# bipul-mohanto/OptixPathTracer

Measured on AMD Instinct MI355X. Metric: Mrays/s (and ms/frame) at 1080p 4spp depth8; 1/2/4/8 MI355X scaling, higher is better.
Workload: dtype f32

## Files before the change

### optixpathtracer_amd/csrc/pt_bvh8.h

```cpp
#pragma once
#ifdef PT_BVH8_NODE_ONLY
#include "pt_bvh.h"
#else
#include "pt_kernels.h"
#endif

struct Node8 {
    float4 n0, n1, n2, n3, n4;
};
#ifndef PT8_LEAF_MAX
#define PT8_LEAF_MAX 3
#endif
static_assert(PT8_LEAF_MAX >= 1 && PT8_LEAF_MAX <= 3, "leafbits holds 3 bits per slot");

PT_DEV float u8f(uint32_t v, int k) { return (float)((v >> (8 * k)) & 0xffu); }

struct Bvh8Dev {
    const Node8* nodes;
    const LeafTri* tris;
    float hit_pad;
};

struct NodeHdr {
    float ox, oy, oz, sx, sy, sz;
    uint32_t imask, child_base, tri_base;
    uint32_t lbits;
};
PT_DEV NodeHdr node_hdr(const float4 n0, const float4 n1) {
    NodeHdr n;
    const uint32_t e01 = __float_as_uint(n0.w), e2m = __float_as_uint(n1.w);
    n.ox = n0.x; n.oy = n0.y; n.oz = n0.z;
    n.sx = __uint_as_float(e01 << 16); n.sy = __uint_as_float(e01 & 0xffff0000u); n.sz = __uint_as_float(e2m << 16);
    n.imask = e2m >> 16;
    n.child_base = __float_as_uint(n1.x);
    n.tri_base = __float_as_uint(n1.y);
    n.lbits = __float_as_uint(n1.z);
    return n;
}
PT_DEV uint32_t leaf_pending(uint32_t hm, uint32_t lbits) {
    uint32_t sp3 = (hm | (hm << 8)) & 0x00F00Fu;
    sp3 = (sp3 | (sp3 << 4)) & 0x0C30C3u;
    sp3 = (sp3 | (sp3 << 2)) & 0x249249u;
    return (sp3 * 7u) & lbits;
}
PT_DEV uint32_t leaf_of(uint32_t tri_base, uint32_t lbits, uint32_t bit) { return tri_base + (uint32_t)__popc(lbits & ((1u << bit) - 1u)); }
PT_DEV uint32_t leaf_first(uint32_t tri_base, uint32_t lbits, uint32_t s) { return leaf_of(tri_base, lbits, 3u * s); }
PT_DEV uint32_t leaf_count(uint32_t lbits, uint32_t s) { return (uint32_t)__popc((lbits >> (3u * s)) & 7u); }

#ifndef PT_BVH8_NODE_ONLY
#ifndef PT8_LDS_DEPTH
#define PT8_LDS_DEPTH 10
#endif
#define PT8_OVF_DEPTH 52
#ifndef PT8_REFILL
#define PT8_REFILL 40
#endif
#ifndef PT8_TRI_BIAS
#define PT8_TRI_BIAS 2
#endif
#ifndef PT8_MIN_CHUNK
#define PT8_MIN_CHUNK 64
#endif
#define PT8_CHUNK 512
#ifndef PT8_WAVES_PER_EU
#define PT8_WAVES_PER_EU 5
#endif
#ifndef PT8_STEAL_PERIOD
#define PT8_STEAL_PERIOD 3
#endif

#define PT8_WAVE_SYNC() do { __builtin_amdgcn_fence(__ATOMIC_SEQ_CST, "wavefront"); __builtin_amdgcn_wave_barrier(); } while (0)

#define PT_WAVELOG_CAP (1u << 20)
#ifdef PT_DEBUG_STATS
#define PT_STAT(x) x
#else
#define PT_STAT(x)
#endif
#if defined(PT_DEBUG_STATS) || defined(PT_DEBUG_WAVELOG)
#define PT_WLOG(x) x
#else
#define PT_WLOG(x)
#endif

#define PT_WSTRIDE 16
struct Trace8Args {
    PathState st;
    Bvh8Dev bvh;
    QView queue;
    QView queue2;
    uint32_t* work;
    uint32_t* ovf;
    int cull_back;
    unsigned long long* dbg;
    int bounce;
    int lds_skip;
    int ovf_depth;
    uint32_t* fault;
    uint32_t num_nodes;
};

#if __HIP_DEVICE_COMPILE__
typedef __attribute__((address_space(3))) uint32_t* Lds32;
typedef __attribute__((address_space(1))) uint32_t* Global32;
#else
typedef uint32_t* Lds32;
typedef uint32_t* Global32;
#endif

template <int MODE, bool LOCAL, bool CARRY = false>
PT_DEV void trace8_wave(const Trace8Args& a, const uint32_t wid, const uint32_t nw, const uint32_t ln1, const uint32_t ln2, const uint32_t woff) {
    __shared__ uint32_t s_stack[PT8_LDS_DEPTH * 2 * 64];
    __shared__ uint32_t s_prefix[PT_NSUB + 1];
    __shared__ uint32_t s_prefix2[PT_NSUB + 1];
    __shared__ unsigned long long s_key[64];
    __shared__ uint32_t s_cnt[64];
    __shared__ int32_t s_leaf[64];
    __shared__ uint32_t s_vlane[64];
    const uint32_t lane = threadIdx.x;
    const uint32_t gtid = blockIdx.x * 64u + lane;
    const uint32_t gstride = gridDim.x * 64u;
    const int lds_depth = PT8_LDS_DEPTH - a.lds_skip;
    const uint32_t n1 = LOCAL ? ln1 : qreader_init(a.queue, s_prefix);
    const uint32_t n2 = (MODE == TR_UNIFIED) ? (LOCAL ? ln2 : qreader_init(a.queue2, s_prefix2)) : 0u;
    const uint32_t n = n1 + n2;
    uint32_t chunk = (n / (nw * 2u)) & ~(uint32_t)(PT8_MIN_CHUNK < 64 ? PT8_MIN_CHUNK - 1 : 63);
    chunk = chunk < (uint32_t)PT8_MIN_CHUNK ? (uint32_t)PT8_MIN_CHUNK : (chunk > (uint32_t)PT8_CHUNK ? (uint32_t)PT8_CHUNK : chunk);
    if (LOCAL) chunk = n;
    const bool no_share = (unsigned long long)wid * chunk >= n;
    const uint32_t nchunks = (n + chunk - 1u) / chunk;
    if (no_share) return;
    uint32_t chunk_next = wid * chunk;
    uint32_t chunk_end = (chunk_next + chunk < n) ? chunk_next + chunk : n;
    const unsigned long long lt_mask = (1ull << lane) - 1ull;
    bool shadow_lane = (MODE == TR_SHADOW_APPLY);

    bool active = false, exhausted = false;
    RaySetup r;
    r.o = r.d = r.idir = r.dn = mk3(0.f);
    float tmin = 0.f, tmax = 0.f, best = 0.f;
    int32_t bprim = -1;
    int32_t bleaf = -1;
    uint32_t pm = 0;
    uint32_t g_base = 0, g_imask = 0, g_hits = 0;
    uint32_t t_base = 0, t_mask = 0, t_bits = 0;
    int sp = 0;
    bool stealing = false;
    uint32_t misc = lane;
#define OWNER (misc & 0xffu)
#define SB ((int)(misc >> 24))
#define SET_OWNER(v) (misc = (misc & ~0xffu) | (uint32_t)(v))
#define SET_SB(v) (misc = (misc & 0x00ffffffu) | ((uint32_t)(v) << 24))
    uint32_t slot = 0;
    bool unwritten = false;
    PT_STAT(uint32_t c_nodes = 0; uint32_t c_tris = 0; uint32_t c_maxsp = 0; uint32_t c_push = 0; uint32_t c_ray = 0; uint32_t c_raymax = 0; uint32_t c_iters = 0;
            uint32_t c_act = 0; uint32_t c_exec = 0; uint32_t c_nodeit = 0;)
    PT_WLOG(const unsigned long long w_t0 = wall_clock64(); unsigned long long w_tex = 0; uint32_t w_iters = 0;)
    PT_WLOG(unsigned long long w_cw = 0; unsigned long long w_cr = 0; unsigned long long w_cs = 0; uint32_t w_np = 0;)
    PT_WLOG(unsigned long long w_c01 = 0; unsigned long long w_c12 = 0; unsigned long long w_c23 = 0; const unsigned long long w_c0 = clock64();)

    const char* const node_bytes = reinterpret_cast<const char*>(a.bvh.nodes);
    const char* const tri_bytes = reinterpret_cast<const char*>(a.bvh.tris);
    const Lds32 lds_stack = (Lds32)s_stack;
    const Global32 ovf_stack = (Global32)a.ovf;
    auto push = [&](uint32_t v0, uint32_t v1) {
        PT_STAT(++c_push; if ((uint32_t)sp + 1 > c_maxsp) c_maxsp = sp + 1;)
        if (sp < lds_depth) {
            lds_stack[(sp * 2) * 64 + lane] = v0;
            lds_stack[(sp * 2 + 1) * 64 + lane] = v1;
            ++sp;
        } else if (sp < lds_depth + a.ovf_depth) {
            ovf_stack[(size_t)((sp - lds_depth) * 2) * gstride + gtid] = v0;
            ovf_stack[(size_t)((sp - lds_depth) * 2 + 1) * gstride + gtid] = v1;
            ++sp;
        } else {
            atomicOr(a.fault, 1u);
        }
    };
    auto pop = [&](uint32_t& v0, uint32_t& v1) {
        --sp;
        if (sp < lds_depth) {
            v0 = lds_stack[(sp * 2) * 64 + lane];
            v1 = lds_stack[(sp * 2 + 1) * 64 + lane];
        } else {
            v0 = ovf_stack[(size_t)((sp - lds_depth) * 2) * gstride + gtid];
            v1 = ovf_stack[(size_t)((sp - lds_depth) * 2 + 1) * gstride + gtid];
            __builtin_amdgcn_s_waitcnt(0x0f70);
        }
    };
    auto write_result = [&](float rbest, int32_t rprim) {
        if (MODE == TR_SHADOW_APPLY || (MODE == TR_UNIFIED && shadow_lane)) {
            const bool occluded = rprim != 0;
            if (MODE == TR_UNIFIED && CARRY) {
                st_st<PT_NT_TRACE_ST>(&a.st.svis[slot], occluded ? 0u : 1u);
                return;
            }
            const uint32_t ps = (MODE == TR_UNIFIED ? a.queue2 : a.queue).base[slot];
            if (a.st.vis) {
                if (!occluded) atomicOr(&a.st.vis[ps], 1u << a.bounce);
                return;
            }
            const float4 pe = st_ld<PT_NT_TRACE_LD>(&a.st.shPend[slot]);
            const int kind = __float_as_int(pe.w);
            if (kind == PEND_ALPHA) {
                if (occluded) {
                    const float4 x = a.st.alpha[ps];
                    a.st.alpha[ps] = make_float4(x.x + pe.x, x.y + pe.y, x.z + pe.z, 0.f);
                }
            } else if (!occluded) {
                float4* acc = (kind == PEND_DIRECT) ? a.st.direct : a.st.indirect;
                const float4 x = st_ld<PT_NT_TRACE_LD>(&acc[ps]);
                st_st<PT_NT_TRACE_ST>(&acc[ps], make_float4(x.x + pe.x, x.y + pe.y, x.z + pe.z, 0.f));
            }
        } else {
            st_st<PT_NT_TRACE_ST>(&a.st.hit[slot], make_float2(rbest, __int_as_float(rprim)));
        }
    };
    const auto is_shadow = [&]() { return MODE == TR_SHADOW_APPLY || MODE == TR_ANY_QUERY || (MODE == TR_UNIFIED && shadow_lane); };
    auto local_key = [&]() -> unsigned long long {
        if (is_shadow()) return bprim != 0 ? 0ull : ~0ull;
        return ((unsigned long long)__float_as_uint(best) << 32) | (unsigned long long)(uint32_t)bprim;
    };
    auto finish = [&]() {
        if (stealing) {
            atomicMin(&s_key[OWNER], local_key());
            if (atomicSub(&s_cnt[OWNER], 1u) == 1u) {
                const unsigned long long k = s_key[OWNER];
                if (is_shadow()) write_result(0.f, k == 0ull ? 1 : 0);
                else write_result(__uint_as_float((uint32_t)(k >> 32)), (int32_t)(uint32_t)k < 0 ? -1 : s_leaf[OWNER]);
            }
            active = false;
            return;
        }
        unwritten = true;
        active = false;
        PT_STAT(if (c_ray > c_raymax) c_raymax = c_ray;
                if (a.dbg) atomicAdd(&a.dbg[(is_shadow() ? 32 : 16) + (31 - __clz((int)(c_ray | 1u)))], 1ull);
                c_ray = 0;)
    };

    auto start_ray = [&](float ox, float oy, float oz, float dx, float dy, float dz) {
        r.o = mk3(ox, oy, oz);
        r.d = mk3(dx, dy, dz);
        r.idir = mk3(__builtin_amdgcn_rcpf(dx), __builtin_amdgcn_rcpf(dy), __builtin_amdgcn_rcpf(dz));
        r.dn = scl3(r.d, 1.0f / dot3(r.d, r.d));
        if (!(fabsf(dx) > 1e-30f)) r.idir.x = copysignf(1e30f, dx);
        if (!(fabsf(dy) > 1e-30f)) r.idir.y = copysignf(1e30f, dy);
        if (!(fabsf(dz) > 1e-30f)) r.idir.z = copysignf(1e30f, dz);
        pm = ((__float_as_uint(dz) >> 31) ? 0xF0u : 0x0Fu) | (((__float_as_uint(dy) >> 31) ? 0xCCu : 0x33u) << 8) | (((__float_as_uint(dx) >> 31) ? 0xAAu : 0x55u) << 16);
        sp = 0;
        SET_SB(0);
        t_mask = 0;
    };

    for (;;) {
        PT_WLOG(const unsigned long long w_p0 = clock64(); ++w_np;)
        if (unwritten) {
            write_result(best, is_shadow() ? bprim : bleaf);
            unwritten = false;
        }
        PT_WLOG(__builtin_amdgcn_s_waitcnt(0); const unsigned long long w_p1 = clock64(); w_cw += w_p1 - w_p0;)
        const unsigned long long idle = __ballot(!active);
        if (idle != 0ull && !exhausted) {
            const uint32_t cnt = (uint32_t)__popcll(idle);
            if (chunk_next == chunk_end) {
                if (nchunks <= nw) {
                    exhausted = true;
                } else {
                    uint32_t c = 0;
                    if (lane == 0) c = atomicAdd(a.work, 1u);
                    c = __shfl(c, 0) + nw;
                    const unsigned long long b0 = (unsigned long long)c * chunk;
                    chunk_next = b0 < n ? (uint32_t)b0 : n;
                    chunk_end = (b0 + chunk < n) ? (uint32_t)(b0 + chunk) : n;
                    if (chunk_next >= chunk_end) exhausted = true;
                }
            }
            const uint32_t take = (chunk_end - chunk_next) < cnt ? (chunk_end - chunk_next) : cnt;
            const uint32_t rank = (uint32_t)__popcll(idle & lt_mask);
            const uint32_t first = chunk_next;
            chunk_next += take;
            if (chunk_next == chunk_end && nchunks <= nw) exhausted = true;
            if (!active && rank < take) {
                const uint32_t gi = first + rank;
                if (LOCAL) {
                    shadow_lane = (MODE == TR_SHADOW_APPLY) || (MODE == TR_UNIFIED && gi < n2);
                    slot = woff + ((MODE == TR_UNIFIED && !shadow_lane) ? gi - n2 : gi);
                } else if (MODE == TR_UNIFIED) {
                    shadow_lane = gi < n2;
                    uint32_t hint = shadow_lane ? (misc >> 16) & 0xffu : (misc >> 8) & 0xffu;
                    slot = shadow_lane ? qreader_pos_hint(a.queue2, s_prefix2, gi, hint) : qreader_pos_hint(a.queue, s_prefix, gi - n2, hint);
                    misc = shadow_lane ? (misc & 0xff00ffffu) | (hint << 16) : (misc & 0xffff00ffu) | (hint << 8);
                } else {
                    uint32_t hint = (misc >> 8) & 0xffu;
                    slot = qreader_pos_hint(a.queue, s_prefix, gi, hint);
                    misc = (misc & 0xffff00ffu) | (hint << 8);
                }
                float4 o4, d4;
                if (MODE == TR_SHADOW_APPLY || (MODE == TR_UNIFIED && shadow_lane)) {
                    if (a.st.vis) {
                        const size_t bi = (size_t)a.bounce * a.st.bstride + (MODE == TR_UNIFIED ? a.queue2 : a.queue).base[slot];
                        o4 = a.st.sO[bi];
                        d4 = a.st.sD[bi];
                    } else {
                        o4 = st_ld<PT_NT_TRACE_LD>(&a.st.shO[slot]);
                        d4 = st_ld<PT_NT_TRACE_LD>(&a.st.shD[slot]);
                    }
                    tmin = 0.01f;
                    tmax = 1e16f;
                } else {
                    o4 = st_ld<PT_NT_TRACE_LD>(&a.st.rayO[slot]);
                    d4 = st_ld<PT_NT_TRACE_LD>(&a.st.rayD[slot]);
                    tmin = o4.w;
                    tmax = d4.w;
                }
                start_ray(o4.x, o4.y, o4.z, d4.x, d4.y, d4.z);
                best = tmax;
                bprim = (MODE == TR_CLOSEST || (MODE == TR_UNIFIED && !shadow_lane)) ? -1 : 0;
                bleaf = -1;
                g_base = 0;
                g_imask = 1u;
                g_hits = 1u;
                active = true;
            }
        }
        PT_WLOG(__builtin_amdgcn_s_waitcnt(0); const unsigned long long w_p2 = clock64(); w_cr += w_p2 - w_p1;)
        if (exhausted) {
            if (!stealing) {
                stealing = true;
                PT_WLOG(w_tex = wall_clock64();)
                SET_OWNER(lane);
                if (active) {
                    s_leaf[lane] = bleaf;
                    s_cnt[lane] = 1u;
                    s_key[lane] = local_key();
                }
                PT8_WAVE_SYNC();
            }
            const unsigned long long idle2 = __ballot(!active);
            const bool victim = active && sp > SB && SB < lds_depth;
            const unsigned long long vmask = __ballot(victim);
            if (idle2 != 0ull && vmask != 0ull) {
                const uint32_t ni = (uint32_t)__popcll(idle2), nv = (uint32_t)__popcll(vmask);
                const uint32_t m = ni < nv ? ni : nv;
                const uint32_t vrank = (uint32_t)__popcll(vmask & lt_mask), irank = (uint32_t)__popcll(idle2 & lt_mask);
                const bool give = victim && vrank < m, take = !active && irank < m;
                if (give) s_vlane[vrank] = lane;
                PT8_WAVE_SYNC();
                const uint32_t v = take ? s_vlane[irank] : lane;
                const float ox = __shfl(r.o.x, (int)v), oy = __shfl(r.o.y, (int)v), oz = __shfl(r.o.z, (int)v);
                const float dx = __shfl(r.d.x, (int)v), dy = __shfl(r.d.y, (int)v), dz = __shfl(r.d.z, (int)v);
                const float ix = __shfl(r.idir.x, (int)v), iy = __shfl(r.idir.y, (int)v), iz = __shfl(r.idir.z, (int)v);
                const float nx_ = __shfl(r.dn.x, (int)v), ny_ = __shfl(r.dn.y, (int)v), nz_ = __shfl(r.dn.z, (int)v);
                const float vtmin = __shfl(tmin, (int)v), vtmax = __shfl(tmax, (int)v);
                const uint32_t vpm = __shfl(pm, (int)v), vslot = __shfl(slot, (int)v), vmisc = __shfl(misc, (int)v);
                const uint32_t vowner = vmisc & 0xffu;
                const int vsb = (int)(vmisc >> 24);
                const int vshadow = __shfl((int)shadow_lane, (int)v);
                if (take) {
                    r.o = mk3(ox, oy, oz);
                    r.d = mk3(dx, dy, dz);
                    r.idir = mk3(ix, iy, iz);
                    r.dn = mk3(nx_, ny_, nz_);
                    tmin = vtmin;
                    tmax = vtmax;
                    pm = vpm;
                    slot = vslot;
                    SET_OWNER(vowner);
                    shadow_lane = vshadow != 0;
                    const uint32_t e0 = s_stack[(vsb * 2) * 64 + v], e1 = s_stack[(vsb * 2 + 1) * 64 + v];
                    g_base = e0;
                    g_imask = e1 & 0xffu;
                    g_hits = e1 >> 8;
                    t_mask = 0;
                    sp = 0;
                    SET_SB(0);
                    const unsigned long long k = s_key[OWNER];
                    if (is_shadow()) {
                        best = tmax;
                        bprim = 0;
                    } else {
                        best = __uint_as_float((uint32_t)(k >> 32));
                        bprim = (int32_t)(uint32_t)k;
                    }
                    atomicAdd(&s_cnt[OWNER], 1u);
                    active = true;
                }
                PT8_WAVE_SYNC();
                if (give) {
                    const int nsb = SB + 1;
                    SET_SB(nsb == sp ? 0 : nsb);
                    if (nsb == sp) sp = 0;
                }
            }
        }
        PT_WLOG(w_cs += clock64() - w_p2;)
        unsigned long long act = __ballot(active);
        if (act == 0ull) break;
        const uint32_t thresh = exhausted ? 1u : (uint32_t)PT8_REFILL;
        uint32_t it = 0;
        do {
            if (stealing && active) {
                const unsigned long long k = s_key[OWNER];
                if (is_shadow()) {
                    if (k == 0ull) finish();
                } else if (k < local_key()) {
                    best = __uint_as_float((uint32_t)(k >> 32));
                    bprim = (int32_t)(uint32_t)k;
                }
            }
            PT_WLOG(const unsigned long long w_a = clock64();)
            const bool want_tri = active && t_mask != 0u;
            const bool want_node = active && t_mask == 0u;
            const unsigned long long m_tri = __ballot(want_tri), m_node = __ballot(want_node);
            const bool node_turn = __popcll(m_node) >= PT8_TRI_BIAS * __popcll(m_tri);
            PT_WLOG(unsigned long long w_b = w_a; unsigned long long w_c = w_a;)
            if (want_node && node_turn) {
                if (g_hits == 0u) {
                    if (sp == SB) {
                        finish();
                    } else {
                        uint32_t v0, v1;
                        pop(v0, v1);
                        g_base = v0;
                        g_imask = v1 & 0xffu;
                        g_hits = v1 >> 8;
                    }
                }
                if (active) {
                    uint32_t h = g_hits, t = h & pm;
                    h = t ? t : h;
                    t = h & (pm >> 8);
                    h = t ? t : h;
                    t = h & (pm >> 16);
                    h = t ? t : h;
                    g_hits ^= h;
                    const uint32_t idx = g_base + (uint32_t)__popc(g_imask & (h - 1u));
                    if (g_hits != 0u) push(g_base, g_imask | (g_hits << 8));
                    PT_STAT(++c_nodes; ++c_ray;)
                    const Node8* nd = reinterpret_cast<const Node8*>(node_bytes + idx * (uint32_t)sizeof(Node8));
                    const float4 n0 = nd->n0, n1 = nd->n1, n2 = nd->n2, n3 = nd->n3, n4 = nd->n4;
                    PT_WLOG(w_b = clock64(); __builtin_amdgcn_s_waitcnt(0); w_c = clock64();)
                    const NodeHdr nh = node_hdr(n0, n1);
                    const uint32_t imask = nh.imask;
                    const float ax = nh.sx * r.idir.x, ay = nh.sy * r.idir.y, az = nh.sz * r.idir.z;
                    const float bx = (nh.ox - r.o.x) * r.idir.x, by = (nh.oy - r.o.y) * r.idir.y, bz = (nh.oz - r.o.z) * r.idir.z;
                    const bool nx = r.idir.x < 0.0f, ny = r.idir.y < 0.0f, nz = r.idir.z < 0.0f;
                    const uint32_t lox0 = __float_as_uint(n2.x), lox1 = __float_as_uint(n2.y), loy0 = __float_as_uint(n2.z), loy1 = __float_as_uint(n2.w);
                    const uint32_t loz0 = __float_as_uint(n3.x), loz1 = __float_as_uint(n3.y), hix0 = __float_as_uint(n3.z), hix1 = __float_as_uint(n3.w);
                    const uint32_t hiy0 = __float_as_uint(n4.x), hiy1 = __float_as_uint(n4.y), hiz0 = __float_as_uint(n4.z), hiz1 = __float_as_uint(n4.w);
                    const uint32_t nearx[2] = {nx ? hix0 : lox0, nx ? hix1 : lox1}, farx[2] = {nx ? lox0 : hix0, nx ? lox1 : hix1};
                    const uint32_t neary[2] = {ny ? hiy0 : loy0, ny ? hiy1 : loy1}, fary[2] = {ny ? loy0 : hiy0, ny ? loy1 : hiy1};
                    const uint32_t nearz[2] = {nz ? hiz0 : loz0, nz ? hiz1 : loz1}, farz[2] = {nz ? loz0 : hiz0, nz ? loz1 : hiz1};
                    uint32_t miss = 0u;
#pragma unroll
                    for (int s = 7; s >= 0; --s) {
                        const int w = s >> 2, k = s & 3;
                        const float tnx = __builtin_fmaf(u8f(nearx[w], k), ax, bx), tfx = __builtin_fmaf(u8f(farx[w], k), ax, bx);
                        const float tny = __builtin_fmaf(u8f(neary[w], k), ay, by), tfy = __builtin_fmaf(u8f(fary[w], k), ay, by);
                        const float tnz = __builtin_fmaf(u8f(nearz[w], k), az, bz), tfz = __builtin_fmaf(u8f(farz[w], k), az, bz);
                        const float tn = fmaxf(fmaxf(tnx, tny), fmaxf(tnz, tmin));
                        const float tf = fminf(fminf(tfx, tfy), fminf(tfz, best));
                        miss = __builtin_amdgcn_alignbit(miss, __float_as_uint(tf - tn), 31u);
                    }
                    const uint32_t hm = miss ^ 0xffu;
                    const uint32_t hits = hm & imask;
                    g_base = nh.child_base;
                    g_imask = imask;
                    g_hits = hits;
                    t_base = nh.tri_base;
                    t_bits = nh.lbits;
                    t_mask = leaf_pending(hm, nh.lbits);
                }
            }
            if (want_tri && !node_turn) {
                const uint32_t bit = (uint32_t)__ffs((int)t_mask) - 1u;
                t_mask &= t_mask - 1u;
                PT_STAT(++c_tris; ++c_ray;)
                const uint32_t leaf = leaf_of(t_base, t_bits, bit);
                const LeafTri* tp = reinterpret_cast<const LeafTri*>(tri_bytes + leaf * (uint32_t)sizeof(LeafTri));
                const float4 ta = tp->t0, tb = tp->t1, tc = tp->t2;
                PT_WLOG(w_b = clock64(); __builtin_amdgcn_s_waitcnt(0); w_c = clock64();)
                float t, det;
                const v3 v0 = mk3(ta.x, ta.y, ta.z), v1 = mk3(ta.w, tb.x, tb.y), v2 = mk3(tb.z, tb.w, tc.x);
                if (tri_test_det(r, v0, v1, v2, t, det)) {
                    const int32_t prim = __float_as_int(tc.y);
                    if (MODE == TR_SHADOW_APPLY || MODE == TR_ANY_QUERY || (MODE == TR_UNIFIED && shadow_lane)) {
                        if (t > tmin && t < tmax && (!a.cull_back || det > 0.0f) && hit_in_box(r, v0, v1, v2, a.bvh.hit_pad, t)) {
                            bprim = 1;
                            best = t;
                            finish();
                        }
                    } else if (t > tmin && (t < best || (t == best && bprim >= 0 && prim < bprim)) && hit_in_box(r, v0, v1, v2, a.bvh.hit_pad, t)) {
                        best = t;
                        bprim = prim;
                        bleaf = (int32_t)leaf;
                        if (stealing) {
                            const unsigned long long key = local_key();
                            atomicMin(&s_key[OWNER], key);
                            if (s_key[OWNER] == key) s_leaf[OWNER] = bleaf;
                        }
                    }
                }
            }
            PT_STAT(++c_iters; if (a.dbg && lane == 0) {
                const bool node_step = __popcll(m_node) >= PT8_TRI_BIAS * __popcll(m_tri);
                c_act += (uint32_t)__popcll(m_node | m_tri);
                c_exec += (uint32_t)__popcll(node_step ? m_node : m_tri);
                c_nodeit += node_step ? 1u : 0u;
            })
            PT_WLOG(++w_iters; w_c01 += w_b - w_a; w_c12 += w_c - w_b; w_c23 += clock64() - w_c;)
            act = __ballot(active);
            ++it;
            if (stealing && act != ~0ull && it >= (uint32_t)PT8_STEAL_PERIOD) break;
        } while ((uint32_t)__popcll(act) >= thresh);
    }
    PT_STAT(if (a.dbg) {
        atomicAdd(&a.dbg[0], (unsigned long long)c_nodes);
        atomicAdd(&a.dbg[1], (unsigned long long)c_tris);
        atomicMax(&a.dbg[2], (unsigned long long)c_maxsp);
        atomicAdd(&a.dbg[3], (unsigned long long)c_push);
        atomicMax(&a.dbg[4], (unsigned long long)c_raymax);
        atomicMax(&a.dbg[5], (unsigned long long)c_iters);
        if (lane == 0) {
            atomicAdd(&a.dbg[6], (unsigned long long)c_iters);
            atomicAdd(&a.dbg[7], 1ull);
            atomicAdd(&a.dbg[8], (unsigned long long)c_act);
            atomicAdd(&a.dbg[9], (unsigned long long)c_exec);
            atomicAdd(&a.dbg[10], (unsigned long long)c_nodeit);
        }
    })
    PT_WLOG(if (a.dbg && lane == 0) {
        const unsigned long long k = atomicAdd(&a.dbg[63], 1ull);
        if (k < (unsigned long long)PT_WAVELOG_CAP) {
            unsigned long long* w = a.dbg + 64 + 8 * k;
            w[6] = (w_c01 << 32) | (w_c12 & 0xffffffffull);
            w[7] = (w_c23 << 32) | ((clock64() - w_c0 - w_c01 - w_c12 - w_c23) & 0xffffffffull);
            w[0] = (unsigned long long)(uintptr_t)a.work;
            w[1] = ((unsigned long long)MODE << 32) | n;
            w[2] = w_t0;
            w[3] = wall_clock64();
            w[4] = w_tex;
            w[5] = w_iters;
        }
    })
}
#undef OWNER
#undef SB
#undef SET_OWNER
#undef SET_SB

template <int MODE>
__global__ void __launch_bounds__(64) __attribute__((amdgpu_waves_per_eu(PT8_WAVES_PER_EU, PT8_WAVES_PER_EU)))
k_trace8(Trace8Args a) {
    trace8_wave<MODE, false>(a, blockIdx.x, gridDim.x, 0u, 0u, 0u);
}
__global__ void __launch_bounds__(64) __attribute__((amdgpu_waves_per_eu(PT8_WAVES_PER_EU, PT8_WAVES_PER_EU)))
k_trace8_vis(Trace8Args a) {
    trace8_wave<TR_UNIFIED, false, true>(a, blockIdx.x, gridDim.x, 0u, 0u, 0u);
}

#ifndef PT8_CAM_STACK
#define PT8_CAM_STACK 64
#endif
#if __HIP_DEVICE_COMPILE__
typedef const __attribute__((address_space(4))) Node8* ConstNode8;
typedef const __attribute__((address_space(4))) LeafTri* ConstLeafTri;
#endif
__global__ void __launch_bounds__(64) k_trace8_cam(Trace8Args a) {
#if __HIP_DEVICE_COMPILE__
    __shared__ uint2 s_grp[PT8_CAM_STACK];
    const uint32_t lane = threadIdx.x;
    const uint32_t n = a.queue.counts[0];
    const uint32_t npk = (n + 63u) >> 6;
    uint32_t per = npk / (gridDim.x * 4u);
    per = per < 4u ? 4u : (per > 16u ? 16u : per);
    uint32_t pk = blockIdx.x * per, pk_end = pk + per;
    const ConstNode8 nodes = (ConstNode8)(uintptr_t)a.bvh.nodes;
    const ConstLeafTri tris = (ConstLeafTri)(uintptr_t)a.bvh.tris;
    for (;;) {
        if (pk == pk_end) {
            uint32_t c = 0;
            if (lane == 0) c = atomicAdd(a.work, 1u);
            c = (uint32_t)__builtin_amdgcn_readfirstlane((int)c) + gridDim.x;
            pk = c * per;
            pk_end = pk + per;
        }
        if (pk >= npk) break;
        const uint32_t pos = (pk << 6) + lane;
        ++pk;
        const bool valid = pos < n;
        float4 o4 = make_float4(0.f, 0.f, 0.f, 1.f), d4 = make_float4(0.f, 0.f, 1.f, -1.f);
        if (valid) {
            o4 = st_ld<PT_NT_TRACE_LD>(&a.st.rayO[pos]);
            d4 = st_ld<PT_NT_TRACE_LD>(&a.st.rayD[pos]);
        }
        RaySetup r;
        r.o = mk3(o4.x, o4.y, o4.z);
        r.d = mk3(d4.x, d4.y, d4.z);
        r.idir = mk3(__builtin_amdgcn_rcpf(d4.x), __builtin_amdgcn_rcpf(d4.y), __builtin_amdgcn_rcpf(d4.z));
        r.dn = scl3(r.d, 1.0f / dot3(r.d, r.d));
        if (!(fabsf(d4.x) > 1e-30f)) r.idir.x = copysignf(1e30f, d4.x);
        if (!(fabsf(d4.y) > 1e-30f)) r.idir.y = copysignf(1e30f, d4.y);
        if (!(fabsf(d4.z) > 1e-30f)) r.idir.z = copysignf(1e30f, d4.z);
        const float tmin = o4.w;
        float best = d4.w;
        int32_t bprim = -1, bleaf = -1;
        const uint32_t pm_lane = ((__float_as_uint(d4.z) >> 31) ? 0xF0u : 0x0Fu) | (((__float_as_uint(d4.y) >> 31) ? 0xCCu : 0x33u) << 8) |
                                 (((__float_as_uint(d4.x) >> 31) ? 0xAAu : 0x55u) << 16);
        const uint32_t pm = (uint32_t)__builtin_amdgcn_readfirstlane((int)pm_lane);
        const bool nx = r.idir.x < 0.0f, ny = r.idir.y < 0.0f, nz = r.idir.z < 0.0f;
        uint32_t g_base = 0u, g_imask = 1u, g_hits = 1u;
        int sp = 0;
        PT_STAT(uint32_t c_nodes = 0; uint32_t c_tris = 0; uint32_t c_mine = 0; uint32_t c_hitl = 0;)
        for (;;) {
            if (g_hits == 0u) {
                if (sp == 0) break;
                --sp;
                const uint2 e = s_grp[sp];
                g_base = (uint32_t)__builtin_amdgcn_readfirstlane((int)e.x);
                const uint32_t e1 = (uint32_t)__builtin_amdgcn_readfirstlane((int)e.y);
                g_imask = e1 & 0xffu;
                g_hits = e1 >> 8;
            }
            uint32_t h = g_hits, t = h & pm;
            h = t ? t : h;
            t = h & (pm >> 8);
            h = t ? t : h;
            t = h & (pm >> 16);
            h = t ? t : h;
            g_hits ^= h;
            const uint32_t idx = g_base + (uint32_t)__popc(g_imask & (h - 1u));
            if (g_hits != 0u) {
                if (sp < PT8_CAM_STACK) s_grp[sp] = make_uint2(g_base, g_imask | (g_hits << 8));
                else atomicOr(a.fault, 1u);
                sp = sp < PT8_CAM_STACK ? sp + 1 : sp;
            }
            const float4 n0 = nodes[idx].n0, n1 = nodes[idx].n1, n2 = nodes[idx].n2, n3 = nodes[idx].n3, n4 = nodes[idx].n4;
            const NodeHdr nh = node_hdr(n0, n1);
            const uint32_t imask = nh.imask;
            const float ax = nh.sx * r.idir.x, ay = nh.sy * r.idir.y, az = nh.sz * r.idir.z;
            const float bx = (nh.ox - r.o.x) * r.idir.x, by = (nh.oy - r.o.y) * r.idir.y, bz = (nh.oz - r.o.z) * r.idir.z;
            const uint32_t lox0 = __float_as_uint(n2.x), lox1 = __float_as_uint(n2.y), loy0 = __float_as_uint(n2.z), loy1 = __float_as_uint(n2.w);
            const uint32_t loz0 = __float_as_uint(n3.x), loz1 = __float_as_uint(n3.y), hix0 = __float_as_uint(n3.z), hix1 = __float_as_uint(n3.w);
            const uint32_t hiy0 = __float_as_uint(n4.x), hiy1 = __float_as_uint(n4.y), hiz0 = __float_as_uint(n4.z), hiz1 = __float_as_uint(n4.w);
            const uint32_t nearx[2] = {nx ? hix0 : lox0, nx ? hix1 : lox1}, farx[2] = {nx ? lox0 : hix0, nx ? lox1 : hix1};
            const uint32_t neary[2] = {ny ? hiy0 : loy0, ny ? hiy1 : loy1}, fary[2] = {ny ? loy0 : hiy0, ny ? loy1 : hiy1};
            const uint32_t nearz[2] = {nz ? hiz0 : loz0, nz ? hiz1 : loz1}, farz[2] = {nz ? loz0 : hiz0, nz ? loz1 : hiz1};
            uint32_t miss = 0u;
#pragma unroll
            for (int s = 7; s >= 0; --s) {
                const int w = s >> 2, k = s & 3;
                const float tnx = __builtin_fmaf(u8f(nearx[w], k), ax, bx), tfx = __builtin_fmaf(u8f(farx[w], k), ax, bx);
                const float tny = __builtin_fmaf(u8f(neary[w], k), ay, by), tfy = __builtin_fmaf(u8f(fary[w], k), ay, by);
                const float tnz = __builtin_fmaf(u8f(nearz[w], k), az, bz), tfz = __builtin_fmaf(u8f(farz[w], k), az, bz);
                const float tn = fmaxf(fmaxf(tnx, tny), fmaxf(tnz, tmin));
                const float tf = fminf(fminf(tfx, tfy), fminf(tfz, best));
                miss = __builtin_amdgcn_alignbit(miss, __float_as_uint(tf - tn), 31u);
            }
            const uint32_t hm = miss ^ 0xffu;
            PT_STAT(++c_nodes; c_hitl += (uint32_t)__popcll(__ballot(hm != 0u));)
            uint32_t whm = 0u;
#pragma unroll
            for (int s = 0; s < 8; ++s) whm |= __ballot((hm >> s) & 1u) != 0ull ? (1u << s) : 0u;
            uint32_t lm = whm & ~imask;
            while (lm != 0u) {
                const uint32_t s = (uint32_t)__ffs((int)lm) - 1u;
                lm &= lm - 1u;
                const bool mine = (hm >> s) & 1u;
                const uint32_t cnt = leaf_count(nh.lbits, s), first_leaf = leaf_first(nh.tri_base, nh.lbits, s);
                for (uint32_t k = 0; k < cnt; ++k) {
                    const uint32_t leaf = first_leaf + k;
                    const float4 ta = tris[leaf].t0, tb = tris[leaf].t1, tc = tris[leaf].t2;
                    PT_STAT(++c_tris; c_mine += (uint32_t)__popcll(__ballot(mine));)
                    if (mine) {
                        float tt, det;
                        const v3 v0 = mk3(ta.x, ta.y, ta.z), v1 = mk3(ta.w, tb.x, tb.y), v2 = mk3(tb.z, tb.w, tc.x);
                        if (tri_test_det(r, v0, v1, v2, tt, det)) {
                            const int32_t prim = __float_as_int(tc.y);
                            if (tt > tmin && (tt < best || (tt == best && bprim >= 0 && prim < bprim)) && hit_in_box(r, v0, v1, v2, a.bvh.hit_pad, tt)) {
                                best = tt;
                                bprim = prim;
                                bleaf = (int32_t)leaf;
                            }
                        }
                    }
                }
            }
            g_base = nh.child_base;
            g_imask = imask;
            g_hits = whm & imask;
        }
        if (valid) st_st<PT_NT_TRACE_ST>(&a.st.hit[pos], make_float2(best, __int_as_float(bleaf)));
        PT_STAT(if (a.dbg && lane == 0) {
            atomicAdd(&a.dbg[48], 1ull);
            atomicAdd(&a.dbg[49], (unsigned long long)c_nodes);
            atomicAdd(&a.dbg[50], (unsigned long long)c_tris);
            atomicAdd(&a.dbg[51], (unsigned long long)c_mine);
            atomicAdd(&a.dbg[52], (unsigned long long)c_hitl);
        })
    }
#endif
}
#endif
```

Baseline: 5030.

## Split BVH8 traversal into templated refill and stealing phases with wave-mask state

Restructures the wavefront traversal loop into two separate loops, a refill phase and a work-stealing phase, each running a templated iterate lambda, so the stealing checks are compiled out of the main phase. Per-lane active, unwritten and stealing booleans are replaced by a wave-wide active mask, derived from pm and set via ballot and inverse-ballot, with sp=-1 marking a pending result write. Queue counts are made wave-uniform with readfirstlane so they can sit in scalar registers. The aim is to cut VGPR pressure and divergent branch overhead in the hot loop, at the cost of duplicated code and more complex control flow.

```diff
diff --git a/optixpathtracer_amd/csrc/pt_bvh8.h b/optixpathtracer_amd/csrc/pt_bvh8.h
--- a/optixpathtracer_amd/csrc/pt_bvh8.h
+++ b/optixpathtracer_amd/csrc/pt_bvh8.h
@@ -71,6 +71,11 @@
 
 #define PT8_WAVE_SYNC() do { __builtin_amdgcn_fence(__ATOMIC_SEQ_CST, "wavefront"); __builtin_amdgcn_wave_barrier(); } while (0)
 
+#define PT8_VOTE(cmp) __builtin_amdgcn_ballot_w64(cmp)
+#define PT8_LANE_IN(mask) __builtin_amdgcn_inverse_ballot_w64(mask)
+PT_DEV uint32_t pt8_uniform(uint32_t v) { return (uint32_t)__builtin_amdgcn_readfirstlane((int)v); }
+template <bool STEALING> struct Pt8Phase { static constexpr bool stealing = STEALING; };
+
 #define PT_WAVELOG_CAP (1u << 20)
 #ifdef PT_DEBUG_STATS
 #define PT_STAT(x) x
@@ -121,8 +126,8 @@
     const uint32_t gtid = blockIdx.x * 64u + lane;
     const uint32_t gstride = gridDim.x * 64u;
     const int lds_depth = PT8_LDS_DEPTH - a.lds_skip;
-    const uint32_t n1 = LOCAL ? ln1 : qreader_init(a.queue, s_prefix);
-    const uint32_t n2 = (MODE == TR_UNIFIED) ? (LOCAL ? ln2 : qreader_init(a.queue2, s_prefix2)) : 0u;
+    const uint32_t n1 = pt8_uniform(LOCAL ? ln1 : qreader_init(a.queue, s_prefix));
+    const uint32_t n2 = (MODE == TR_UNIFIED) ? pt8_uniform(LOCAL ? ln2 : qreader_init(a.queue2, s_prefix2)) : 0u;
     const uint32_t n = n1 + n2;
     uint32_t chunk = (n / (nw * 2u)) & ~(uint32_t)(PT8_MIN_CHUNK < 64 ? PT8_MIN_CHUNK - 1 : 63);
     chunk = chunk < (uint32_t)PT8_MIN_CHUNK ? (uint32_t)PT8_MIN_CHUNK : (chunk > (uint32_t)PT8_CHUNK ? (uint32_t)PT8_CHUNK : chunk);
@@ -135,7 +140,7 @@
     const unsigned long long lt_mask = (1ull << lane) - 1ull;
     bool shadow_lane = (MODE == TR_SHADOW_APPLY);
 
-    bool active = false, exhausted = false;
+    unsigned long long act = 0ull;
     RaySetup r;
     r.o = r.d = r.idir = r.dn = mk3(0.f);
     float tmin = 0.f, tmax = 0.f, best = 0.f;
@@ -145,14 +150,12 @@
     uint32_t g_base = 0, g_imask = 0, g_hits = 0;
     uint32_t t_base = 0, t_mask = 0, t_bits = 0;
     int sp = 0;
-    bool stealing = false;
     uint32_t misc = lane;
 #define OWNER (misc & 0xffu)
 #define SB ((int)(misc >> 24))
 #define SET_OWNER(v) (misc = (misc & ~0xffu) | (uint32_t)(v))
 #define SET_SB(v) (misc = (misc & 0x00ffffffu) | ((uint32_t)(v) << 24))
     uint32_t slot = 0;
-    bool unwritten = false;
     PT_STAT(uint32_t c_nodes = 0; uint32_t c_tris = 0; uint32_t c_maxsp = 0; uint32_t c_push = 0; uint32_t c_ray = 0; uint32_t c_raymax = 0; uint32_t c_iters = 0;
             uint32_t c_act = 0; uint32_t c_exec = 0; uint32_t c_nodeit = 0;)
     PT_WLOG(const unsigned long long w_t0 = wall_clock64(); unsigned long long w_tex = 0; uint32_t w_iters = 0;)
@@ -165,13 +168,16 @@
     const Global32 ovf_stack = (Global32)a.ovf;
     auto push = [&](uint32_t v0, uint32_t v1) {
         PT_STAT(++c_push; if ((uint32_t)sp + 1 > c_maxsp) c_maxsp = sp + 1;)
-        if (sp < lds_depth) {
+        if (__builtin_expect(sp < lds_depth, 1)) {
             lds_stack[(sp * 2) * 64 + lane] = v0;
             lds_stack[(sp * 2 + 1) * 64 + lane] = v1;
             ++sp;
-        } else if (sp < lds_depth + a.ovf_depth) {
-            ovf_stack[(size_t)((sp - lds_depth) * 2) * gstride + gtid] = v0;
-            ovf_stack[(size_t)((sp - lds_depth) * 2 + 1) * gstride + gtid] = v1;
+            return;
+        }
+        const int lv = sp - lds_depth;
+        if (lv < a.ovf_depth) {
+            ovf_stack[(size_t)(lv * 2) * gstride + gtid] = v0;
+            ovf_stack[(size_t)(lv * 2 + 1) * gstride + gtid] = v1;
             ++sp;
         } else {
             atomicOr(a.fault, 1u);
@@ -221,19 +227,18 @@
         if (is_shadow()) return bprim != 0 ? 0ull : ~0ull;
         return ((unsigned long long)__float_as_uint(best) << 32) | (unsigned long long)(uint32_t)bprim;
     };
-    auto finish = [&]() {
-        if (stealing) {
+    auto finish = [&](auto phase) {
+        pm = 0u;
+        if (decltype(phase)::stealing) {
             atomicMin(&s_key[OWNER], local_key());
             if (atomicSub(&s_cnt[OWNER], 1u) == 1u) {
                 const unsigned long long k = s_key[OWNER];
                 if (is_shadow()) write_result(0.f, k == 0ull ? 1 : 0);
                 else write_result(__uint_as_float((uint32_t)(k >> 32)), (int32_t)(uint32_t)k < 0 ? -1 : s_leaf[OWNER]);
             }
-            active = false;
             return;
         }
-        unwritten = true;
-        active = false;
+        sp = -1;
         PT_STAT(if (c_ray > c_raymax) c_raymax = c_ray;
                 if (a.dbg) atomicAdd(&a.dbg[(is_shadow() ? 32 : 16) + (31 - __clz((int)(c_ray | 1u)))], 1ull);
                 c_ray = 0;)
@@ -253,15 +258,133 @@
         t_mask = 0;
     };
 
+    auto iterate = [&](auto phase) {
+        constexpr bool STEALING = decltype(phase)::stealing;
+        if (STEALING) {
+            if (PT8_LANE_IN(act)) {
+                const unsigned long long k = s_key[OWNER];
+                if (is_shadow()) {
+                    if (k == 0ull) finish(phase);
+                } else if (k < local_key()) {
+                    best = __uint_as_float((uint32_t)(k >> 32));
+                    bprim = (int32_t)(uint32_t)k;
+                }
+            }
+            act = PT8_VOTE(pm != 0u);
+        }
+        PT_WLOG(const unsigned long long w_a = clock64();)
+        const unsigned long long m_pend = PT8_VOTE(t_mask != 0u);
+        const unsigned long long m_tri = act & m_pend, m_node = act & ~m_pend;
+        const bool node_turn = __popcll(m_node) >= PT8_TRI_BIAS * __popcll(m_tri);
+        PT_WLOG(unsigned long long w_b = w_a; unsigned long long w_c = w_a;)
+        if (PT8_LANE_IN(node_turn ? m_node : 0ull)) {
+            if (g_hits == 0u) {
+                if (sp == SB) {
+                    finish(phase);
+                } else {
+                    uint32_t v0, v1;
+                    pop(v0, v1);
+                    g_base = v0;
+                    g_imask = v1 & 0xffu;
+                    g_hits = v1 >> 8;
+                }
+            }
+            if (pm != 0u) {
+                uint32_t h = g_hits, t = h & pm;
+                h = t ? t : h;
+                t = h & (pm >> 8);
+                h = t ? t : h;
+                t = h & (pm >> 16);
+                h = t ? t : h;
+                g_hits ^= h;
+                const uint32_t idx = g_base + (uint32_t)__popc(g_imask & (h - 1u));
+                if (g_hits != 0u) push(g_base, g_imask | (g_hits << 8));
+                PT_STAT(++c_nodes; ++c_ray;)
+                const Node8* nd = reinterpret_cast<const Node8*>(node_bytes + idx * (uint32_t)sizeof(Node8));
+                const float4 n0 = nd->n0, n1 = nd->n1, n2 = nd->n2, n3 = nd->n3, n4 = nd->n4;
+                PT_WLOG(w_b = clock64(); __builtin_amdgcn_s_waitcnt(0); w_c = clock64();)
+                const NodeHdr nh = node_hdr(n0, n1);
+                const uint32_t imask = nh.imask;
+                const float ax = nh.sx * r.idir.x, ay = nh.sy * r.idir.y, az = nh.sz * r.idir.z;
+                const float bx = (nh.ox - r.o.x) * r.idir.x, by = (nh.oy - r.o.y) * r.idir.y, bz = (nh.oz - r.o.z) * r.idir.z;
+                const bool nx = r.idir.x < 0.0f, ny = r.idir.y < 0.0f, nz = r.idir.z < 0.0f;
+                const uint32_t lox0 = __float_as_uint(n2.x), lox1 = __float_as_uint(n2.y), loy0 = __float_as_uint(n2.z), loy1 = __float_as_uint(n2.w);
+                const uint32_t loz0 = __float_as_uint(n3.x), loz1 = __float_as_uint(n3.y), hix0 = __float_as_uint(n3.z), hix1 = __float_as_uint(n3.w);
+                const uint32_t hiy0 = __float_as_uint(n4.x), hiy1 = __float_as_uint(n4.y), hiz0 = __float_as_uint(n4.z), hiz1 = __float_as_uint(n4.w);
+                const uint32_t nearx[2] = {nx ? hix0 : lox0, nx ? hix1 : lox1}, farx[2] = {nx ? lox0 : hix0, nx ? lox1 : hix1};
+                const uint32_t neary[2] = {ny ? hiy0 : loy0, ny ? hiy1 : loy1}, fary[2] = {ny ? loy0 : hiy0, ny ? loy1 : hiy1};
+                const uint32_t nearz[2] = {nz ? hiz0 : loz0, nz ? hiz1 : loz1}, farz[2] = {nz ? loz0 : hiz0, nz ? loz1 : hiz1};
+                uint32_t miss = 0u;
+#pragma unroll
+                for (int s = 7; s >= 0; --s) {
+                    const int w = s >> 2, k = s & 3;
+                    const float tnx = __builtin_fmaf(u8f(nearx[w], k), ax, bx), tfx = __builtin_fmaf(u8f(farx[w], k), ax, bx);
+                    const float tny = __builtin_fmaf(u8f(neary[w], k), ay, by), tfy = __builtin_fmaf(u8f(fary[w], k), ay, by);
+                    const float tnz = __builtin_fmaf(u8f(nearz[w], k), az, bz), tfz = __builtin_fmaf(u8f(farz[w], k), az, bz);
+                    const float tn = fmaxf(fmaxf(tnx, tny), fmaxf(tnz, tmin));
+                    const float tf = fminf(fminf(tfx, tfy), fminf(tfz, best));
+                    miss = __builtin_amdgcn_alignbit(miss, __float_as_uint(tf - tn), 31u);
+                }
+                const uint32_t hm = miss ^ 0xffu;
+                const uint32_t hits = hm & imask;
+                g_base = nh.child_base;
+                g_imask = imask;
+                g_hits = hits;
+                t_base = nh.tri_base;
+                t_bits = nh.lbits;
+                t_mask = leaf_pending(hm, nh.lbits);
+            }
+        }
+        if (PT8_LANE_IN(node_turn ? 0ull : m_tri)) {
+            const uint32_t bit = (uint32_t)__ffs((int)t_mask) - 1u;
+            t_mask &= t_mask - 1u;
+            PT_STAT(++c_tris; ++c_ray;)
+            const uint32_t leaf = leaf_of(t_base, t_bits, bit);
+            const LeafTri* tp = reinterpret_cast<const LeafTri*>(tri_bytes + leaf * (uint32_t)sizeof(LeafTri));
+            const float4 ta = tp->t0, tb = tp->t1, tc = tp->t2;
+            PT_WLOG(w_b = clock64(); __builtin_amdgcn_s_waitcnt(0); w_c = clock64();)
+            float t, det;
+            const v3 v0 = mk3(ta.x, ta.y, ta.z), v1 = mk3(ta.w, tb.x, tb.y), v2 = mk3(tb.z, tb.w, tc.x);
+            if (tri_test_det(r, v0, v1, v2, t, det)) {
+                const int32_t prim = __float_as_int(tc.y);
+                if (MODE == TR_SHADOW_APPLY || MODE == TR_ANY_QUERY || (MODE == TR_UNIFIED && shadow_lane)) {
+                    if (t > tmin && t < tmax && (!a.cull_back || det > 0.0f) && hit_in_box(r, v0, v1, v2, a.bvh.hit_pad, t)) {
+                        bprim = 1;
+                        best = t;
+                        finish(phase);
+                    }
+                } else if (t > tmin && (t < best || (t == best && bprim >= 0 && prim < bprim)) && hit_in_box(r, v0, v1, v2, a.bvh.hit_pad, t)) {
+                    best = t;
+                    bprim = prim;
+                    bleaf = (int32_t)leaf;
+                    if (STEALING) {
+                        const unsigned long long key = local_key();
+                        atomicMin(&s_key[OWNER], key);
+                        if (s_key[OWNER] == key) s_leaf[OWNER] = bleaf;
+                    }
+                }
+            }
+        }
+        PT_STAT(++c_iters; if (a.dbg && lane == 0) {
+            const bool node_step = __popcll(m_node) >= PT8_TRI_BIAS * __popcll(m_tri);
+            c_act += (uint32_t)__popcll(m_node | m_tri);
+            c_exec += (uint32_t)__popcll(node_step ? m_node : m_tri);
+            c_nodeit += node_step ? 1u : 0u;
+        })
+        PT_WLOG(++w_iters; w_c01 += w_b - w_a; w_c12 += w_c - w_b; w_c23 += clock64() - w_c;)
+        act = PT8_VOTE(pm != 0u);
+    };
+
     for (;;) {
+        bool exhausted = false;
         PT_WLOG(const unsigned long long w_p0 = clock64(); ++w_np;)
-        if (unwritten) {
+        if (sp < 0) {
             write_result(best, is_shadow() ? bprim : bleaf);
-            unwritten = false;
+            sp = 0;
         }
         PT_WLOG(__builtin_amdgcn_s_waitcnt(0); const unsigned long long w_p1 = clock64(); w_cw += w_p1 - w_p0;)
-        const unsigned long long idle = __ballot(!active);
-        if (idle != 0ull && !exhausted) {
+        const unsigned long long idle = ~act;
+        if (idle != 0ull) {
             const uint32_t cnt = (uint32_t)__popcll(idle);
             if (chunk_next == chunk_end) {
                 if (nchunks <= nw) {
@@ -269,7 +392,7 @@
                 } else {
                     uint32_t c = 0;
                     if (lane == 0) c = atomicAdd(a.work, 1u);
-                    c = __shfl(c, 0) + nw;
+                    c = pt8_uniform(c) + nw;
                     const unsigned long long b0 = (unsigned long long)c * chunk;
                     chunk_next = b0 < n ? (uint32_t)b0 : n;
                     chunk_end = (b0 + chunk < n) ? (uint32_t)(b0 + chunk) : n;
@@ -281,7 +404,7 @@
             const uint32_t first = chunk_next;
             chunk_next += take;
             if (chunk_next == chunk_end && nchunks <= nw) exhausted = true;
-            if (!active && rank < take) {
+            if (PT8_LANE_IN(idle & PT8_VOTE(rank < take))) {
                 const uint32_t gi = first + rank;
                 if (LOCAL) {
                     shadow_lane = (MODE == TR_SHADOW_APPLY) || (MODE == TR_UNIFIED && gi < n2);
@@ -321,199 +444,89 @@
                 g_base = 0;
                 g_imask = 1u;
                 g_hits = 1u;
-                active = true;
-            }
+            }
+            act = PT8_VOTE(pm != 0u);
         }
         PT_WLOG(__builtin_amdgcn_s_waitcnt(0); const unsigned long long w_p2 = clock64(); w_cr += w_p2 - w_p1;)
-        if (exhausted) {
-            if (!stealing) {
-                stealing = true;
-                PT_WLOG(w_tex = wall_clock64();)
-                SET_OWNER(lane);
-                if (active) {
-                    s_leaf[lane] = bleaf;
-                    s_cnt[lane] = 1u;
-                    s_key[lane] = local_key();
-                }
-                PT8_WAVE_SYNC();
-            }
-            const unsigned long long idle2 = __ballot(!active);
-            const bool victim = active && sp > SB && SB < lds_depth;
-            const unsigned long long vmask = __ballot(victim);
-            if (idle2 != 0ull && vmask != 0ull) {
-                const uint32_t ni = (uint32_t)__popcll(idle2), nv = (uint32_t)__popcll(vmask);
-                const uint32_t m = ni < nv ? ni : nv;
-                const uint32_t vrank = (uint32_t)__popcll(vmask & lt_mask), irank = (uint32_t)__popcll(idle2 & lt_mask);
-                const bool give = victim && vrank < m, take = !active && irank < m;
-                if (give) s_vlane[vrank] = lane;
-                PT8_WAVE_SYNC();
-                const uint32_t v = take ? s_vlane[irank] : lane;
-                const float ox = __shfl(r.o.x, (int)v), oy = __shfl(r.o.y, (int)v), oz = __shfl(r.o.z, (int)v);
-                const float dx = __shfl(r.d.x, (int)v), dy = __shfl(r.d.y, (int)v), dz = __shfl(r.d.z, (int)v);
-                const float ix = __shfl(r.idir.x, (int)v), iy = __shfl(r.idir.y, (int)v), iz = __shfl(r.idir.z, (int)v);
-                const float nx_ = __shfl(r.dn.x, (int)v), ny_ = __shfl(r.dn.y, (int)v), nz_ = __shfl(r.dn.z, (int)v);
-                const float vtmin = __shfl(tmin, (int)v), vtmax = __shfl(tmax, (int)v);
-                const uint32_t vpm = __shfl(pm, (int)v), vslot = __shfl(slot, (int)v), vmisc = __shfl(misc, (int)v);
-                const uint32_t vowner = vmisc & 0xffu;
-                const int vsb = (int)(vmisc >> 24);
-                const int vshadow = __shfl((int)shadow_lane, (int)v);
-                if (take) {
-                    r.o = mk3(ox, oy, oz);
-                    r.d = mk3(dx, dy, dz);
-                    r.idir = mk3(ix, iy, iz);
-                    r.dn = mk3(nx_, ny_, nz_);
-                    tmin = vtmin;
-                    tmax = vtmax;
-                    pm = vpm;
-                    slot = vslot;
-                    SET_OWNER(vowner);
-                    shadow_lane = vshadow != 0;
-                    const uint32_t e0 = s_stack[(vsb * 2) * 64 + v], e1 = s_stack[(vsb * 2 + 1) * 64 + v];
-                    g_base = e0;
-                    g_imask = e1 & 0xffu;
-                    g_hits = e1 >> 8;
-                    t_mask = 0;
-                    sp = 0;
-                    SET_SB(0);
-                    const unsigned long long k = s_key[OWNER];
-                    if (is_shadow()) {
-                        best = tmax;
-                        bprim = 0;
-                    } else {
-                        best = __uint_as_float((uint32_t)(k >> 32));
-                        bprim = (int32_t)(uint32_t)k;
-                    }
-                    atomicAdd(&s_cnt[OWNER], 1u);
-                    active = true;
-                }
-                PT8_WAVE_SYNC();
-                if (give) {
-                    const int nsb = SB + 1;
-                    SET_SB(nsb == sp ? 0 : nsb);
-                    if (nsb == sp) sp = 0;
-                }
-            }
-        }
+        if (exhausted || act == 0ull) break;
         PT_WLOG(w_cs += clock64() - w_p2;)
-        unsigned long long act = __ballot(active);
+        do iterate(Pt8Phase<false>()); while ((uint32_t)__popcll(act) >= (uint32_t)PT8_REFILL);
+    }
+
+    PT_WLOG(w_tex = wall_clock64();)
+    SET_OWNER(lane);
+    if (PT8_LANE_IN(act)) {
+        s_leaf[lane] = bleaf;
+        s_cnt[lane] = 1u;
+        s_key[lane] = local_key();
+    }
+    PT8_WAVE_SYNC();
+    for (;;) {
+        PT_WLOG(const unsigned long long w_s0 = clock64(); ++w_np;)
+        const bool active = PT8_LANE_IN(act);
+        const unsigned long long idle2 = ~act;
+        const bool victim = active && sp > SB && SB < lds_depth;
+        const unsigned long long vmask = __ballot(victim);
+        if (idle2 != 0ull && vmask != 0ull) {
+            const uint32_t ni = (uint32_t)__popcll(idle2), nv = (uint32_t)__popcll(vmask);
+            const uint32_t m = ni < nv ? ni : nv;
+            const uint32_t vrank = (uint32_t)__popcll(vmask & lt_mask), irank = (uint32_t)__popcll(idle2 & lt_mask);
+            const bool give = victim && vrank < m, take = !active && irank < m;
+            if (give) s_vlane[vrank] = lane;
+            PT8_WAVE_SYNC();
+            const uint32_t v = take ? s_vlane[irank] : lane;
+            const float ox = __shfl(r.o.x, (int)v), oy = __shfl(r.o.y, (int)v), oz = __shfl(r.o.z, (int)v);
+            const float dx = __shfl(r.d.x, (int)v), dy = __shfl(r.d.y, (int)v), dz = __shfl(r.d.z, (int)v);
+            const float ix = __shfl(r.idir.x, (int)v), iy = __shfl(r.idir.y, (int)v), iz = __shfl(r.idir.z, (int)v);
+            const float nx_ = __shfl(r.dn.x, (int)v), ny_ = __shfl(r.dn.y, (int)v), nz_ = __shfl(r.dn.z, (int)v);
+            const float vtmin = __shfl(tmin, (int)v), vtmax = __shfl(tmax, (int)v);
+            const uint32_t vpm = __shfl(pm, (int)v), vslot = __shfl(slot, (int)v), vmisc = __shfl(misc, (int)v);
+            const uint32_t vowner = vmisc & 0xffu;
+            const int vsb = (int)(vmisc >> 24);
+            const int vshadow = __shfl((int)shadow_lane, (int)v);
+            if (take) {
+                r.o = mk3(ox, oy, oz);
+                r.d = mk3(dx, dy, dz);
+                r.idir = mk3(ix, iy, iz);
+                r.dn = mk3(nx_, ny_, nz_);
+                tmin = vtmin;
+                tmax = vtmax;
+                pm = vpm;
+                slot = vslot;
+                SET_OWNER(vowner);
+                shadow_lane = vshadow != 0;
+                const uint32_t e0 = s_stack[(vsb * 2) * 64 + v], e1 = s_stack[(vsb * 2 + 1) * 64 + v];
+                g_base = e0;
+                g_imask = e1 & 0xffu;
+                g_hits = e1 >> 8;
+                t_mask = 0;
+                sp = 0;
+                SET_SB(0);
+                const unsigned long long k = s_key[OWNER];
+                if (is_shadow()) {
+                    best = tmax;
+                    bprim = 0;
+                } else {
+                    best = __uint_as_float((uint32_t)(k >> 32));
+                    bprim = (int32_t)(uint32_t)k;
+                }
+                atomicAdd(&s_cnt[OWNER], 1u);
+            }
+            PT8_WAVE_SYNC();
+            if (give) {
+                const int nsb = SB + 1;
+                SET_SB(nsb == sp ? 0 : nsb);
+                if (nsb == sp) sp = 0;
+            }
+        }
+        PT_WLOG(w_cs += clock64() - w_s0;)
+        act = PT8_VOTE(pm != 0u);
         if (act == 0ull) break;
-        const uint32_t thresh = exhausted ? 1u : (uint32_t)PT8_REFILL;
         uint32_t it = 0;
         do {
-            if (stealing && active) {
-                const unsigned long long k = s_key[OWNER];
-                if (is_shadow()) {
-                    if (k == 0ull) finish();
-                } else if (k < local_key()) {
-                    best = __uint_as_float((uint32_t)(k >> 32));
-                    bprim = (int32_t)(uint32_t)k;
-                }
-            }
-            PT_WLOG(const unsigned long long w_a = clock64();)
-            const bool want_tri = active && t_mask != 0u;
-            const bool want_node = active && t_mask == 0u;
-            const unsigned long long m_tri = __ballot(want_tri), m_node = __ballot(want_node);
-            const bool node_turn = __popcll(m_node) >= PT8_TRI_BIAS * __popcll(m_tri);
-            PT_WLOG(unsigned long long w_b = w_a; unsigned long long w_c = w_a;)
-            if (want_node && node_turn) {
-                if (g_hits == 0u) {
-                    if (sp == SB) {
-                        finish();
-                    } else {
-                        uint32_t v0, v1;
-                        pop(v0, v1);
-                        g_base = v0;
-                        g_imask = v1 & 0xffu;
-                        g_hits = v1 >> 8;
-                    }
-                }
-                if (active) {
-                    uint32_t h = g_hits, t = h & pm;
-                    h = t ? t : h;
-                    t = h & (pm >> 8);
-                    h = t ? t : h;
-                    t = h & (pm >> 16);
-                    h = t ? t : h;
-                    g_hits ^= h;
-                    const uint32_t idx = g_base + (uint32_t)__popc(g_imask & (h - 1u));
-                    if (g_hits != 0u) push(g_base, g_imask | (g_hits << 8));
-                    PT_STAT(++c_nodes; ++c_ray;)
-                    const Node8* nd = reinterpret_cast<const Node8*>(node_bytes + idx * (uint32_t)sizeof(Node8));
-                    const float4 n0 = nd->n0, n1 = nd->n1, n2 = nd->n2, n3 = nd->n3, n4 = nd->n4;
-                    PT_WLOG(w_b = clock64(); __builtin_amdgcn_s_waitcnt(0); w_c = clock64();)
-                    const NodeHdr nh = node_hdr(n0, n1);
-                    const uint32_t imask = nh.imask;
-                    const float ax = nh.sx * r.idir.x, ay = nh.sy * r.idir.y, az = nh.sz * r.idir.z;
-                    const float bx = (nh.ox - r.o.x) * r.idir.x, by = (nh.oy - r.o.y) * r.idir.y, bz = (nh.oz - r.o.z) * r.idir.z;
-                    const bool nx = r.idir.x < 0.0f, ny = r.idir.y < 0.0f, nz = r.idir.z < 0.0f;
-                    const uint32_t lox0 = __float_as_uint(n2.x), lox1 = __float_as_uint(n2.y), loy0 = __float_as_uint(n2.z), loy1 = __float_as_uint(n2.w);
-                    const uint32_t loz0 = __float_as_uint(n3.x), loz1 = __float_as_uint(n3.y), hix0 = __float_as_uint(n3.z), hix1 = __float_as_uint(n3.w);
-                    const uint32_t hiy0 = __float_as_uint(n4.x), hiy1 = __float_as_uint(n4.y), hiz0 = __float_as_uint(n4.z), hiz1 = __float_as_uint(n4.w);
-                    const uint32_t nearx[2] = {nx ? hix0 : lox0, nx ? hix1 : lox1}, farx[2] = {nx ? lox0 : hix0, nx ? lox1 : hix1};
-                    const uint32_t neary[2] = {ny ? hiy0 : loy0, ny ? hiy1 : loy1}, fary[2] = {ny ? loy0 : hiy0, ny ? loy1 : hiy1};
-                    const uint32_t nearz[2] = {nz ? hiz0 : loz0, nz ? hiz1 : loz1}, farz[2] = {nz ? loz0 : hiz0, nz ? loz1 : hiz1};
-                    uint32_t miss = 0u;
-#pragma unroll
-                    for (int s = 7; s >= 0; --s) {
-                        const int w = s >> 2, k = s & 3;
-                        const float tnx = __builtin_fmaf(u8f(nearx[w], k), ax, bx), tfx = __builtin_fmaf(u8f(farx[w], k), ax, bx);
-                        const float tny = __builtin_fmaf(u8f(neary[w], k), ay, by), tfy = __builtin_fmaf(u8f(fary[w], k), ay, by);
-                        const float tnz = __builtin_fmaf(u8f(nearz[w], k), az, bz), tfz = __builtin_fmaf(u8f(farz[w], k), az, bz);
-                        const float tn = fmaxf(fmaxf(tnx, tny), fmaxf(tnz, tmin));
-                        const float tf = fminf(fminf(tfx, tfy), fminf(tfz, best));
-                        miss = __builtin_amdgcn_alignbit(miss, __float_as_uint(tf - tn), 31u);
-                    }
-                    const uint32_t hm = miss ^ 0xffu;
-                    const uint32_t hits = hm & imask;
-                    g_base = nh.child_base;
-                    g_imask = imask;
-                    g_hits = hits;
-                    t_base = nh.tri_base;
-                    t_bits = nh.lbits;
-                    t_mask = leaf_pending(hm, nh.lbits);
-                }
-            }
-            if (want_tri && !node_turn) {
-                const uint32_t bit = (uint32_t)__ffs((int)t_mask) - 1u;
-                t_mask &= t_mask - 1u;
-                PT_STAT(++c_tris; ++c_ray;)
-                const uint32_t leaf = leaf_of(t_base, t_bits, bit);
-                const LeafTri* tp = reinterpret_cast<const LeafTri*>(tri_bytes + leaf * (uint32_t)sizeof(LeafTri));
-                const float4 ta = tp->t0, tb = tp->t1, tc = tp->t2;
-                PT_WLOG(w_b = clock64(); __builtin_amdgcn_s_waitcnt(0); w_c = clock64();)
-                float t, det;
-                const v3 v0 = mk3(ta.x, ta.y, ta.z), v1 = mk3(ta.w, tb.x, tb.y), v2 = mk3(tb.z, tb.w, tc.x);
-                if (tri_test_det(r, v0, v1, v2, t, det)) {
-                    const int32_t prim = __float_as_int(tc.y);
-                    if (MODE == TR_SHADOW_APPLY || MODE == TR_ANY_QUERY || (MODE == TR_UNIFIED && shadow_lane)) {
-                        if (t > tmin && t < tmax && (!a.cull_back || det > 0.0f) && hit_in_box(r, v0, v1, v2, a.bvh.hit_pad, t)) {
-                            bprim = 1;
-                            best = t;
-                            finish();
-                        }
-                    } else if (t > tmin && (t < best || (t == best && bprim >= 0 && prim < bprim)) && hit_in_box(r, v0, v1, v2, a.bvh.hit_pad, t)) {
-                        best = t;
-                        bprim = prim;
-                        bleaf = (int32_t)leaf;
-                        if (stealing) {
-                            const unsigned long long key = local_key();
-                            atomicMin(&s_key[OWNER], key);
-                            if (s_key[OWNER] == key) s_leaf[OWNER] = bleaf;
-                        }
-                    }
-                }
-            }
-            PT_STAT(++c_iters; if (a.dbg && lane == 0) {
-                const bool node_step = __popcll(m_node) >= PT8_TRI_BIAS * __popcll(m_tri);
-                c_act += (uint32_t)__popcll(m_node | m_tri);
-                c_exec += (uint32_t)__popcll(node_step ? m_node : m_tri);
-                c_nodeit += node_step ? 1u : 0u;
-            })
-            PT_WLOG(++w_iters; w_c01 += w_b - w_a; w_c12 += w_c - w_b; w_c23 += clock64() - w_c;)
-            act = __ballot(active);
-            ++it;
-            if (stealing && act != ~0ull && it >= (uint32_t)PT8_STEAL_PERIOD) break;
-        } while ((uint32_t)__popcll(act) >= thresh);
+            iterate(Pt8Phase<true>());
+            if (++it >= (uint32_t)PT8_STEAL_PERIOD && act != ~0ull) break;
+        } while (act != 0ull);
     }
     PT_STAT(if (a.dbg) {
         atomicAdd(&a.dbg[0], (unsigned long long)c_nodes);
```

After: 5250, median of 6. +4.4%, better.
